# yuzhou42/disinfect-slam

Hardware: AMD Instinct MI355X
Metric: TSDF integrate frames/s (640x480 depth+label, 5mm voxel) (higher is better)
Workload: dtype f32

## Files before the change

### disinfect-slam_amd/csrc/tsdf_device.h

```cpp
#pragma once

#include <hip/hip_runtime.h>
#include <stdint.h>


namespace tsdf {

constexpr int kBlockLenBits = 3;
constexpr int kBlockLen = 8;
constexpr int kBlockVolume = 512;
constexpr int kBlockVolumeBits = 9;
constexpr int kNumBucketBits = 21;
constexpr uint32_t kNumBucket = 1u << kNumBucketBits;
constexpr uint32_t kBucketMask = kNumBucket - 1;
constexpr uint32_t kNumEntry = kNumBucket * 2;
constexpr uint32_t kEntryMask = kNumEntry - 1;
constexpr uint32_t kOccWords = kNumEntry / 64;
constexpr int kBlockBytes = kBlockVolume * 12;
constexpr int kProbOffset = kBlockVolume * 4;
constexpr int kRgbwOffset = kBlockVolume * 8;
constexpr uint32_t kNewKeyCap = 1u << 17;
constexpr int kMaxDdaSamples = 6;
constexpr int64_t kMaxOrderRange = 8192ll * 1024;
constexpr int kResolveThreads = 1024;
// ... 424 lines not shown
  const float u = quot_for_cmp(hx, hz, rz, (float)(P.W - 1));
  const float v = quot_for_cmp(hy, hz, rz, (float)(P.H - 1));
  return u >= 0 && u <= (float)(P.W - 1) && v >= 0 && v <= (float)(P.H - 1) && hz >= 0;
}
template <bool Full>
__device__ __forceinline__ bool block_visible(const FrameParams& P, int16_t bx, int16_t by,
                                              int16_t bz) {
  const int16_t x = (int16_t)(bx << kBlockLenBits), y = (int16_t)(by << kBlockLenBits),
                z = (int16_t)(bz << kBlockLenBits);
  bool vis = Full;
#pragma unroll
  for (int i = 0; i < 8; ++i) {
    const bool v = voxel_visible(P, (int16_t)(x + ((i >> 0) & 1) * (kBlockLen - 1)),
                                 (int16_t)(y + ((i >> 1) & 1) * (kBlockLen - 1)),
                                 (int16_t)(z + ((i >> 2) & 1) * (kBlockLen - 1)));
    if (Full)
      vis = vis && v;
    else
      vis = vis || v;
  }
  return vis;
}

__device__ __forceinline__ f3 pixel_ray(const FrameParams& P, int x, int y) {
  f3 pc;
  pc.x = P.ifx * (float)x + P.icx * 1.0f;
  pc.y = P.ify * (float)y + P.icy * 1.0f;
  pc.z = 1.0f;
  return pc;
}
__device__ __forceinline__ float pixel_w_new(const FrameParams& P, float d) {
  return (1.0f - quot_const(d, P.max_depth, P.inv_max_depth)) * 4.0f;
}

}
```

### disinfect-slam_amd/csrc/tsdf_fuse.hip

```cpp
#include "tsdf_block.h"
#include "tsdf_kernels.h"
#include "tsdf_resolve.h"
#include "tsdf_ingest.h"

namespace tsdf {

__device__ __forceinline__ float comp(const float4& v, int j) {
  return j == 0 ? v.x : j == 1 ? v.y : j == 2 ? v.z : v.w;
}
__device__ __forceinline__ void setc(float4& v, int j, float f) {
  if (j == 0) v.x = f; else if (j == 1) v.y = f; else if (j == 2) v.z = f; else v.w = f;
}
__device__ __forceinline__ uint32_t compu(const uint4& v, int j) {
  return j == 0 ? v.x : j == 1 ? v.y : j == 2 ? v.z : v.w;
}
__device__ __forceinline__ void setu(uint4& v, int j, uint32_t f) {
  if (j == 0) v.x = f; else if (j == 1) v.y = f; else if (j == 2) v.z = f; else v.w = f;
}

__device__ __forceinline__ void frame_end(const EngineDev& D) {
  lds_barrier();
  if (threadIdx.x == 0) {
    D.ctr->total_visible += (unsigned long long)D.ctr->n_vis;
    D.ctr->total_updated += D.ctr->last_updated;
// ... 47 lines not shown

__global__ __launch_bounds__(256) void k_shard_abort(EngineDev D) {
  const int n = min(D.ctr->nk_count, (int)kNewKeyCap);
  for (int i = threadIdx.x; i < n; i += blockDim.x) {
    const int h = (int)D.nk_list[i].slot;
    D.nk_key[h] = 0ull;
    D.nk_order[h] = 0xFFFFFFFFu;
  }
  for (int i = threadIdx.x; i < 3 * kBands; i += blockDim.x) D.band[i * kBandStride] = 0;
  if (threadIdx.x < 2) D.pipe[kPipeNCand + 16 * threadIdx.x] = 0ull;
  for (int i = kPipeStats + threadIdx.x; i < kPipeWords; i += blockDim.x) D.pipe[i] = 0ull;
  for (int i = threadIdx.x; i < kArriveWords; i += blockDim.x) D.arrive[i] = 0ull;
  __syncthreads();
  if (threadIdx.x == 0) {
    D.ctr->nk_count = 0;
    *D.ncand = 0;
    D.ctr->n_fresh = 0;
    D.ctr->n_pend = 0;
    D.ctr->status |= 32u;
  }
}

struct ViewFuse {
  FrameParams R;
  ViewGrid V;
  uint32_t vtag;
};
__device__ __forceinline__ void view_patch_carved(const EngineDev& D, const ViewFuse& F) {
  __builtin_amdgcn_s_waitcnt(0);
  __syncthreads();
  const ViewGrid& V = F.V;
  const int n = min(ld_co(D.ncand), D.cand_cap);
  const int ox = view_origin(F.R.wt.x, F.R.voxel, V.half), oy = view_origin(F.R.wt.y, F.R.voxel, V.half),
            oz = view_origin(F.R.wt.z, F.R.voxel, V.half);
  const unsigned long long* rq = reinterpret_cast<const unsigned long long*>(D.cand);
  for (int k = threadIdx.x; k < n; k += blockDim.x) {
    const unsigned long long a = ld_co(&rq[2 * k]), b = ld_co(&rq[2 * k + 1]);
    const int lx = (int16_t)(a & 0xFFFF) - ox, ly = (int16_t)((a >> 16) & 0xFFFF) - oy,
              lz = (int16_t)((a >> 32) & 0xFFFF) - oz;
    const int32_t idx = (int32_t)(uint32_t)b;
    if ((unsigned)lx >= (unsigned)V.n || (unsigned)ly >= (unsigned)V.n || (unsigned)lz >= (unsigned)V.n || idx < 0)
      continue;
    if (__hip_atomic_load(&D.rtag[idx], __ATOMIC_RELAXED, __HIP_MEMORY_SCOPE_AGENT) != F.vtag) continue;
    const int kb = ((lz >> 2) * V.nb + (ly >> 2)) * V.nb + (lx >> 2);
    __hip_atomic_store(&V.cell[view_cell(kb, lx, ly, lz)], 0u, __ATOMIC_RELAXED, __HIP_MEMORY_SCOPE_AGENT);
  }
}
__device__ __forceinline__ void integrate_tail(const EngineDev& D, const FrameParams& P, DeleteLds& L,
                                               const ViewFuse* F = nullptr) {
  const int t = threadIdx.x;
  const unsigned long long tend = __builtin_amdgcn_s_memrealtime();
  TSDF_STAMP(D, 7, 0);
  if (P.tail == kTailPack)
    pack_cands_wg(D, D.cand, D.ncand, P.slot, P.slot_cap);
  else
    resolve_delete_wg(D, D.cand, D.ncand, 0, L, F ? F->vtag : 0u);
#ifndef TSDF_NO_VIEW_PATCH
  if (F) view_patch_carved(D, *F);
#endif
  TSDF_STAMP(D, 7, 1);
  lds_barrier();
  const int bc = t < kBands ? D.band[t * kBandStride] : 0;
  int nband;
  (void)wg_excl_scan(bc, L.scan, &nband);
  if (t == 0) {
    const unsigned long long upd = arrive_collect(D.arrive + kArrIntegrate);
    D.ctr->last_updated = upd;
    D.ctr->integrate_ticks += tend - ld_co(&D.arrive[kArrStart]);
    D.ctr->n_vis = nband + D.ctr->n_fresh;
  }
  if (P.tail != kTailPack) frame_end(D);
  TSDF_STAMP(D, 7, 2);
}

struct UpdState {
  float4 ts, pr;
  uint4 cw;
  float4 px[4];
  uint32_t pc[4];
  v2f hzs[2];
  bool inb[4];
  bool fresh;
};

__device__ __forceinline__ void update_issue_pool(const EngineDev& D, const VisRec& r, int lane, int hf,
                                                  UpdState& S) {
  const int off = (hf * 256 + lane * 4) * 4;
  const int32_t pidx = r.idx;
  uint8_t* blk = D.pool + (size_t)pidx * kBlockBytes;
  float4& ts = S.ts;
  float4& pr = S.pr;
  uint4& cw = S.cw;
  const bool fresh = r.pad != 0;
  if (fresh) {
    ts = make_float4(-1.f, -1.f, -1.f, -1.f);
    pr = make_float4(0.5f, 0.5f, 0.5f, 0.5f);
    cw = make_uint4(0u, 0u, 0u, 0u);
  } else {
    ts = pool_ld(blk + off);
    pr = pool_ld(blk + kProbOffset + off);
    cw = pool_ldu(blk + kRgbwOffset + off);
  }
  S.fresh = fresh;
}
template <bool Raw>
__device__ __forceinline__ void update_issue_pix(const EngineDev& D, const FrameParams& P, const VisRec& r, int lane,
                                                 int hf, UpdState& S) {
  const int rx0 = (lane & 1) * 4, ry = (lane >> 1) & 7, rz = (lane >> 4) + 4 * hf;
  float4* px = S.px;
  uint32_t* pc = S.pc;
  v2f* hzs = S.hzs;
  bool* inb = S.inb;
  const int16_t ax0 = (int16_t)(r.x << kBlockLenBits), ay = (int16_t)((r.y << kBlockLenBits) + ry),
                az = (int16_t)((r.z << kBlockLenBits) + rz);
  const float fy = (float)ay * P.voxel, fz = (float)az * P.voxel;
  const float qx = P.cq.x, qy = P.cq.y, qz = P.cq.z, qw = P.cq.w;
  const float qx_fz = qx * fz, qx_fy = qx * fy;
  float uvx = qy * fz - qz * fy;
  uvx += uvx;
  const float w_uvx = qw * uvx, qz_uvx = qz * uvx, qy_uvx = qy * uvx;
#pragma unroll
  for (int k = 0; k < 2; ++k) {
    const v2f wx = v2((float)(int16_t)(ax0 + rx0 + 2 * k), (float)(int16_t)(ax0 + rx0 + 2 * k + 1)) * P.voxel;
    v2f uvy = qz * wx - qx_fz;
    v2f uvz = qx_fy - qy * wx;
    uvy += uvy;
    uvz += uvz;
    const v2f cx = qy * uvz - qz * uvy;
    const v2f cy = qz_uvx - qx * uvz;
    const v2f cz = qx * uvy - qy_uvx;
    const v2f pcx = ((wx + w_uvx) + cx) + P.ct.x;
    const v2f pcy = ((fy + qw * uvy) + cy) + P.ct.y;
    const v2f pcz = ((fz + qw * uvz) + cz) + P.ct.z;
    const v2f hx = P.fx * pcx + P.cx * pcz;
    const v2f hy = P.fy * pcy + P.cy * pcz;
    const v2f rz = v2(__builtin_amdgcn_rcpf(pcz.x), __builtin_amdgcn_rcpf(pcz.y));
    int u0, u1, v0, v1;
    round_quot_i2(hx, pcz, rz, true, true, u0, u1);
    round_quot_i2(hy, pcz, rz, true, true, v0, v1);
    hzs[k] = pcz;
    const int uu[2] = {u0, u1}, vv[2] = {v0, v1};
#pragma unroll
    for (int e = 0; e < 2; ++e) {
      const int j = 2 * k + e;
      inb[j] = uu[e] >= 0 && uu[e] < P.W && vv[e] >= 0 && vv[e] < P.H;
      const int img = inb[j] ? vv[e] * P.W + uu[e] : 0;
      if (Raw) {
        pc[j] = (uint32_t)P.rgb[3 * img] | ((uint32_t)P.rgb[3 * img + 1] << 8) |
                ((uint32_t)P.rgb[3 * img + 2] << 16);
        px[j] = make_float4(P.depth[img], P.ht ? P.ht[img] : 1.0f, P.lt ? P.lt[img] : 1.0f,
                            __int_as_float((uu[e] & 0xFFFF) | (vv[e] << 16)));
      } else {
        px[j] = D.pixA[P.pix_off + img];
        pc[j] = D.pixC[P.pix_off + img];
      }
    }
  }
}

template <bool Raw>
__device__ __forceinline__ void update_issue(const EngineDev& D, const FrameParams& P, const VisRec& r, int lane,
                                             int hf, UpdState& S) {
  update_issue_pool(D, r, lane, hf, S);
  update_issue_pix<Raw>(D, P, r, lane, hf, S);
}

template <bool Raw>
__device__ __forceinline__ void update_finish(const EngineDev& D, const FrameParams& P, const VisRec& r, int lane,
                                              int hf, UpdState& S, float& mn, int& my_upd) {
  const int off = (hf * 256 + lane * 4) * 4;
  const float neg_trunc = -P.trunc;
  uint8_t* blk = D.pool + (size_t)r.idx * kBlockBytes;
  float4 ts = S.ts, pr = S.pr;
  uint4 cw = S.cw;
  const float4* px = S.px;
  const uint32_t* pc = S.pc;
  const v2f* hzs = S.hzs;
  const bool* inb = S.inb;
  const bool fresh = S.fresh;
  int upd_mask = 0;
  const uint32_t wold4 = (compu(cw, 0) >> 24) | ((compu(cw, 1) >> 24) << 8) | ((compu(cw, 2) >> 24) << 16) |
                         ((compu(cw, 3) >> 24) << 24);
  float wn[4] = {0.f, 0.f, 0.f, 0.f};
  int pfast = 0;
  v2f lnh2[2], lnl2[2];
#pragma unroll
  for (int k = 0; k < 2; ++k) {
    const int j0 = 2 * k, j1 = 2 * k + 1;
    const v2f d = v2(px[j0].x, px[j1].x);
    v2f rng, w_new = v2(0.f, 0.f), lnh, lnl;
    bool pf0, pf1;
    if (Raw) {
      const int w0 = __float_as_int(px[j0].w), w1 = __float_as_int(px[j1].w);
      const f3 r0 = pixel_ray(P, w0 & 0xFFFF, w0 >> 16);
      const f3 r1 = pixel_ray(P, w1 & 0xFFFF, w1 >> 16);
      rng = v2(sqrtf(dot3(r0, r0)), sqrtf(dot3(r1, r1)));
      w_new = v2(pixel_w_new(P, d.x), pixel_w_new(P, d.y));
      lnh = sem_logf2(v2(px[j0].y, px[j1].y));
      lnl = sem_logf2(v2(px[j0].z, px[j1].z));
      pf0 = sem_pixel_fast(px[j0].y, px[j0].z, d.x, P.max_depth);
      pf1 = sem_pixel_fast(px[j1].y, px[j1].z, d.y, P.max_depth);
    } else {
      rng = v2(fabsf(px[j0].y), fabsf(px[j1].y));
      pf0 = px[j0].y > 0.0f;
      pf1 = px[j1].y > 0.0f;
      lnh = v2(px[j0].z, px[j1].z);
      lnl = v2(px[j0].w, px[j1].w);
    }
    const uint32_t n0 = pc[j0], n1 = pc[j1];
    const v2f sdf = rng * (d - hzs[k]);
    const bool a0 = inb[j0] && !(d.x == 0 || d.x > P.max_depth) && sdf.x > neg_trunc;
    const bool a1 = inb[j1] && !(d.y == 0 || d.y > P.max_depth) && sdf.y > neg_trunc;
    if (a0 || a1) {
      if (!Raw) w_new = (v2(1.0f, 1.0f) - quot_const2(d, P.max_depth, P.inv_max_depth, a0, a1)) * v2(4.0f, 4.0f);
      v2f tn = quot_const2(sdf, P.trunc, P.inv_trunc, a0, a1);
      tn = v2(fminf(1.0f, tn.x), fminf(1.0f, tn.y));
      const uint32_t o0 = compu(cw, j0), o1 = compu(cw, j1);
      const v2f w_old = v2((float)(o0 >> 24), (float)(o1 >> 24));
      const v2f wc = w_old + w_new;
      const v2f iwc = v2(__builtin_amdgcn_rcpf(wc.x), __builtin_amdgcn_rcpf(wc.y));
      uint32_t c0 = 0, c1 = 0;
#pragma unroll
      for (int ch = 0; ch < 3; ++ch) {
        const v2f num = v2((float)((o0 >> (8 * ch)) & 0xFF), (float)((o1 >> (8 * ch)) & 0xFF)) * w_old +
                        v2((float)((n0 >> (8 * ch)) & 0xFF), (float)((n1 >> (8 * ch)) & 0xFF)) * w_new;
        int32_t r0, r1;
        round_quot_pos2(num, wc, iwc, a0, a1, r0, r1);
        c0 |= (uint32_t)min(255, r0) << (8 * ch);
        c1 |= (uint32_t)min(255, r1) << (8 * ch);
      }
      const v2f tnum = v2(comp(ts, j0), comp(ts, j1)) * w_old + tn * w_new;
      const v2f tq = div_pair(tnum, wc, iwc, a0, a1);
      const v2f wr = wc + v2(0x1.fffffep-2f, 0x1.fffffep-2f);
      c0 |= weight_round_cap(wr.x, 40u) << 24;
      c1 |= weight_round_cap(wr.y, 40u) << 24;
      wn[j0] = w_new.x;
      wn[j1] = w_new.y;
      if (a0) {
// ... 39 lines not shown
        const float w_old = (float)((wold4 >> (8 * j)) & 0xFF);
        pn = sem_update_exact(pv, w_old, wn[j], w_old + wn[j], lnh2[j >> 1][j & 1], lnl2[j >> 1][j & 1]);
      }
      setc(pr, j, pn);
    }
  }
  if (upd_mask == 0xF || fresh) {
    pool_st(blk + off, ts);
    pool_st(blk + kProbOffset + off, pr);
    pool_stu(blk + kRgbwOffset + off, cw);
  } else if (upd_mask) {
#pragma unroll
    for (int j = 0; j < 4; ++j)
      if (upd_mask & (1 << j)) {
        reinterpret_cast<float*>(blk + off)[j] = comp(ts, j);
        reinterpret_cast<float*>(blk + kProbOffset + off)[j] = comp(pr, j);
        reinterpret_cast<uint32_t*>(blk + kRgbwOffset + off)[j] = compu(cw, j);
      }
  }
  my_upd += __popc(upd_mask);
}

template <bool Raw>
__device__ __forceinline__ void update_block(const EngineDev& D, const FrameParams& P, const VisRec& r, int lane,
                                             int hf, float& mn, int& my_upd) {
  UpdState S;
  update_issue<Raw>(D, P, r, lane, hf, S);
  update_finish<Raw>(D, P, r, lane, hf, S, mn, my_upd);
}

__device__ __forceinline__ int band_starts_p(const int32_t* band, int lane, int* total) {
  const int c = lane < kBands ? band[lane * kBandStride] : 0;
  int incl = c;
#pragma unroll
  for (int o = 1; o < kBands; o <<= 1) {
    const int n = __shfl_up(incl, o, 64);
    if (lane >= o) incl += n;
  }
  *total = __builtin_amdgcn_readlane(incl, kBands - 1);
  return incl - c;
}
__device__ __forceinline__ int band_starts(const EngineDev& D, int lane, int* total) {
  return band_starts_p(D.band, lane, total);
}
__device__ __forceinline__ size_t band_find_n(int nblocks, int bst, int lane, int b) {
  const unsigned long long m = __ballot(lane < kBands && b >= bst);
  const int bd = __popcll(m) - 1;
  const int ofs = b - __builtin_amdgcn_readlane(bst, bd);
  return (size_t)bd * nblocks + (size_t)__builtin_amdgcn_readfirstlane(ofs);
}
__device__ __forceinline__ size_t band_find(const EngineDev& D, int bst, int lane, int b) {
  return band_find_n(D.nblocks, bst, lane, b);
}

#ifndef TSDF_INTEGRATE_WAVES
#define TSDF_INTEGRATE_WAVES 6
#endif
template <bool Graph, bool Raw>
__device__ __forceinline__ bool integrate_body(const EngineDev& D, const FrameParams& Pv,
                                               const FrameArgs* __restrict__ A, int nint, DeleteLds& L,
                                               int narrive = 0, const ViewFuse* F = nullptr) {
  FrameParams P = Graph ? A->P : Pv;
  if (Graph && A->cands_out) {
    P.tail = kTailPack;
    P.slot = A->cands_out;
    P.slot_cap = A->cand_cap;
  } else if (Graph) {
    P.tail = kTailResolve;
  }
  __shared__ float s_min[4];
  __shared__ int s_upd[4];
  __shared__ int s_last;
  __shared__ int s_ncand, s_ovf;
  __shared__ VisRec s_cand[kIntegrateCandBuf];
  const int lane = lane_id();
  const int wave = __builtin_amdgcn_readfirstlane(threadIdx.x >> 6);
  const int pair = wave >> 1, hf = wave & 1;
  int nvis = 0;
  const int bst = band_starts(D, lane, &nvis);
  const int nband = nvis;
  nvis += D.ctr->n_fresh;
  const int g = blockIdx.x & 7, ngrp = nint >> 3;
  int my_upd = 0;
  if (threadIdx.x == 0) {
    s_ncand = 0;
    s_ovf = 0;
  }
  TSDF_STAMP(D, 3, 0);
  if (blockIdx.x == 0 && threadIdx.x == 0) st_co(&D.arrive[kArrStart], (unsigned long long)__builtin_amdgcn_s_memrealtime());
  const int npairs = (nvis + 1) >> 1;
  const int p_lo = (int)(((long long)npairs * g) >> 3), p_hi = (int)(((long long)npairs * (g + 1)) >> 3);
  for (int pp = p_lo + (blockIdx.x >> 3); pp < p_hi; pp += ngrp) {
    const int b = 2 * pp + pair;
    float mn = __builtin_nanf("");
    VisRec r{};
    if (b < nvis) {
      if (b >= nband) {
        r = D.fresh_vis[b - nband];
      } else {
        r = D.vis[band_find(D, bst, lane, b)];
      }
      update_block<Raw>(D, P, r, lane, hf, mn, my_upd);
    }
    mn = wave_min_u(mn);
    if (lane == 0) s_min[wave] = mn;
    lds_barrier();
    if (hf == 0 && lane == 0 && b < nvis) {
      const float m2 = fminf(s_min[wave], s_min[wave + 1]);
      if (m2 >= 0.9f) {
        const int k = atomicAdd(&s_ncand, 1);
        if (k < kIntegrateCandBuf) {
          s_cand[k] = r;
        } else {
          const int kg = atomicAdd(D.ncand, 1);
          st_rec_co(&D.cand[kg], r);
          s_ovf = 1;
        }
      }
    }
    lds_barrier();
  }
  const int tot = wave_sum(my_upd);
  if (lane == 0) s_upd[wave] = tot;
  lds_barrier();
  const unsigned long long wg_upd = (unsigned long long)(s_upd[0] + s_upd[1] + s_upd[2] + s_upd[3]);
  const int nc = min(s_ncand, kIntegrateCandBuf);
  if (wave == 0 && nc > 0) {
    int k0 = 0;
    if (lane == 0) k0 = atomicAdd(D.ncand, nc);
    k0 = __shfl(k0, 0, 64);
    if (lane < nc) st_rec_co(&D.cand[k0 + lane], s_cand[lane]);
  }
  TSDF_STAMP(D, 3, 1);
#ifdef TSDF_DIAG_STAMPS
  if (threadIdx.x == 0 && D.dbg && blockIdx.x < (unsigned)kDiagMaxWg) {
    unsigned hw, xcc;
    asm volatile("s_getreg_b32 %0, hwreg(HW_REG_HW_ID)" : "=s"(hw));
    asm volatile("s_getreg_b32 %0, hwreg(HW_REG_XCC_ID)" : "=s"(xcc));
    unsigned long long* q = D.dbg + ((size_t)3 * kDiagMaxWg + blockIdx.x) * kDiagStamps;
    q[4] = hw;
    q[5] = xcc;
    q[6] = (unsigned long long)((p_hi - (p_lo + (int)(blockIdx.x >> 3)) + ngrp - 1) / ngrp);
  }
#endif
  const bool drain = (wave == 0 && nc > 0) || (s_ovf && (wave & 1) == 0);
  if (!arrive_last(D.arrive + kArrIntegrate, wg_upd, &s_last, drain, (uint32_t)(narrive ? narrive : nint)))
    return false;
  integrate_tail(D, P, L, F);
  return true;
}

template <bool Graph, bool Raw>
__global__ __launch_bounds__(kIntegrateThreads)
__attribute__((amdgpu_waves_per_eu(TSDF_INTEGRATE_WAVES, TSDF_INTEGRATE_WAVES))) void k_integrate_t(
    EngineDev D, FrameParams Pv, const FrameArgs* __restrict__ A) {
  __shared__ DeleteLds L;
  integrate_body<Graph, Raw>(D, Pv, A, (int)gridDim.x, L);
}

template <bool Graph>
__device__ __forceinline__ void integrate_vg(const EngineDev& D, const FrameParams& Pv, const FrameArgs* A,
                                             const FrameParams& R, const ViewGrid& V, uint32_t vtag, int nint,
                                             DeleteLds& L) {
  const ViewFuse F{R, V, vtag};
  const int narr = (int)gridDim.x;
  if ((int)blockIdx.x < nint) {
    integrate_body<Graph, false>(D, Pv, A, nint, L, narr, &F);
    return;
  }
  const int w = ((int)blockIdx.x - nint) * 256 + (int)threadIdx.x;
  if (V.n && threadIdx.x < 256) {
    const int ox = view_origin(R.wt.x, R.voxel, V.half), oy = view_origin(R.wt.y, R.voxel, V.half),
              oz = view_origin(R.wt.z, R.voxel, V.half);
    unsigned long long occ = D.occ[w];
    while (occ) {
      const int b = __ffsll((long long)occ) - 1;
      occ &= occ - 1;
      const Ent en = load_ent(D.table, (uint32_t)(w * 64 + b));
      const int lx = en.x - ox, ly = en.y - oy, lz = en.z - oz;
      if ((unsigned)lx >= (unsigned)V.n || (unsigned)ly >= (unsigned)V.n || (unsigned)lz >= (unsigned)V.n ||
          !local_idx(en.idx))
        continue;
      const int k = ((lz >> 2) * V.nb + (ly >> 2)) * V.nb + (lx >> 2);
      __hip_atomic_store(&V.cell[view_cell(k, lx, ly, lz)], (V.gen << kViewIdxBits) | (uint32_t)en.idx,
                         __ATOMIC_RELAXED, __HIP_MEMORY_SCOPE_AGENT);
      V.flags[k] = 1;
      V.flags[V.nbw * 32 + ((lz >> 4) * V.ns + (ly >> 4)) * V.ns + (lx >> 4)] = 1;
    }
  }
  __shared__ int s_last;
  if (!arrive_last(D.arrive + kArrIntegrate, 0ull, &s_last, true, (uint32_t)narr)) return;
  if (Graph) {
    FrameParams P = A->P;
    P.tail = kTailResolve;
    integrate_tail(D, P, L, &F);
  } else {
    integrate_tail(D, Pv, L, &F);
  }
}
__global__ __launch_bounds__(kIntegrateThreads)
__attribute__((amdgpu_waves_per_eu(TSDF_INTEGRATE_WAVES, TSDF_INTEGRATE_WAVES))) void k_integrate_vg(
    EngineDev D, FrameParams Pv, FrameParams R, ViewGrid V, uint32_t vtag, int nint) {
  __shared__ DeleteLds L;
  integrate_vg<false>(D, Pv, nullptr, R, V, vtag, nint, L);
}
__global__ __launch_bounds__(kIntegrateThreads)
__attribute__((amdgpu_waves_per_eu(TSDF_INTEGRATE_WAVES, TSDF_INTEGRATE_WAVES))) void k_integrate_vg_g(
    EngineDev D, const FrameArgs* __restrict__ A, int nint) {
  __shared__ DeleteLds L;
  integrate_vg<true>(D, FrameParams{}, A, A->R, A->V, A->vtag, nint, L);
}


__device__ __forceinline__ void pipe_frame_stats(const EngineDev& D, uint32_t f) {
  const int t = threadIdx.x;
  if (t >= 64) return;
  unsigned long long* base = D.pipe + kPipeStats + (size_t)(f & 1u) * (kPipeStatLines * 16);
  const unsigned long long w = base[16 * t], te = base[16 * t + 1];
  base[16 * t] = 0ull;
  base[16 * t + 1] = 0ull;
  unsigned long long vis = w >> 40, upd = w & ((1ull << 40) - 1ull), tmax = te;
#pragma unroll
  for (int o = 32; o > 0; o >>= 1) {
    vis += __shfl_xor(vis, o, 64);
    upd += __shfl_xor(upd, o, 64);
    const unsigned long long m = __shfl_xor(tmax, o, 64);
    tmax = m > tmax ? m : tmax;
  }
  if (t == 0) {
    const unsigned long long t0 = D.pipe[kPipeT0 + 16 * (f & 1u)];
    D.ctr->n_vis = (int32_t)vis;
    D.ctr->last_updated = upd;
    D.ctr->total_visible += vis;
// ... 280 lines not shown
      __builtin_amdgcn_s_sleep(TSDF_PIPE_SLEEP);
      if (++n > (1u << 22)) {
        atomicOr(status, 64u);
        break;
      }
    }
  }
}
__device__ __forceinline__ bool lane_kept(uint32_t* rtag, int32_t idx, uint32_t fc) {
  return __hip_atomic_fetch_or(&rtag[idx], 0u, __ATOMIC_RELAXED, __HIP_MEMORY_SCOPE_AGENT) != fc;
}
__device__ __forceinline__ void pipe_update(const EngineDev& D, const FrameParams& P, const PipeArgs& A, int kind, int wi,
                                            PipeUpdLds& L) {
  int* s_upd = L.upd;
  int* s_vis = L.vis;
  int& s_ncand = L.ncand;
  VisRec* s_cand = L.cand;
  VisRec* s_def = L.def;
  VisRec* s_list = L.list;
  const int lane = lane_id();
  const int wave = __builtin_amdgcn_readfirstlane(threadIdx.x >> 6);
  const int pair = wave >> 1, hf = wave & 1;
  const bool t0 = threadIdx.x == 0;
  const uint32_t fb = A.fid_alloc, fc = A.fid_carve;
  const VisRec* vis = D.vis + (size_t)(fb & 1u) * kBands * (size_t)D.nblocks;
  VisRec* cand = D.cand + (size_t)(fb & 1u) * (size_t)D.cand_cap;
  int32_t* ncand = reinterpret_cast<int32_t*>(D.pipe + kPipeNCand + 16 * (fb & 1u));
  const unsigned long long* carved = D.pipe + kPipeCarved + (blockIdx.x & 7) * 16;
  if (t0) s_ncand = 0;
  if (kind == 0 && wi == 0 && t0)
    st_co(D.pipe + kPipeT0 + 16 * (fb & 1u), (unsigned long long)__builtin_amdgcn_s_memrealtime());
  int bst = 0;
  int nvis = 0, nband = 0, p = 0, p_hi = 0, pstep = 1;
  bool carved_known = false;
  if (kind == 0) {
    bst = band_starts_p(D.band + (size_t)(fb % 3u) * kBands * kBandStride, lane, &nvis);
    nband = nvis;
    if (A.fresh_ready) nvis += D.ctr->n_fresh;
    const int g = wi & 7, npairs = (nvis + 1) >> 1;
    p = (int)(((long long)npairs * g) >> 3) + (wi >> 3);
    p_hi = (int)(((long long)npairs * (g + 1)) >> 3);
    pstep = A.nint >> 3;
  } else {
    wait_tag(D.pipe + kPipeAlloc + (blockIdx.x & 7) * 16, A.tag, &D.ctr->status);
    nvis = ld_co(&D.ctr->n_fresh);
    p = wi;
    p_hi = (nvis + 1) >> 1;
    pstep = kPipeFreshWG;
  }
  const bool chk = A.has_carve && kind == 0;
  const uint32_t* ct = D.ctag + (size_t)(fc & 1u) * D.nblocks;
  int my_upd = 0, my_vis = 0, ndef = 0;
  bool def_done = false;
  const bool fresh_co = kind != 0;
  int& s_n = L.n;
  int& s_ndef = L.ndef;
  float* s_pmin = L.pmin;
  int* s_pdone = L.pdone;
  uint32_t& s_fb = L.fb;
  if (t0) s_fb = fb;
  const unsigned long long lt_mask = (1ull << lane) - 1ull;
  if (t0) s_ndef = 0;
  for (;;) {
    int n = 0;
    lds_barrier();
    if (p < p_hi) {
      const int npr = min((p_hi - p + pstep - 1) / pstep, kPipeList / 2);
      if (wave == 0) {
        const int b = 2 * (p + (lane >> 1) * pstep) + (lane & 1);
        const bool valid = lane < 2 * npr && b < nvis;
        int bd = 0, bs = 0;
#pragma unroll
        for (int k = 1; k < kBands; ++k) {
          const int sk = __builtin_amdgcn_readlane(bst, k);
          if (b >= sk) {
            bd = k;
            bs = sk;
          }
        }
        VisRec r{};
        if (valid) {
          if (b >= nband)
            r = fresh_co ? ld_rec_co(&D.fresh_vis[b - nband]) : D.fresh_vis[b - nband];
          else
            r = vis[(size_t)bd * D.nblocks + (size_t)(b - bs)];
        }
        const bool cand = valid && chk && r.pad == 0 && ct[r.idx] == fc;
        bool take = valid && !cand;
        const unsigned long long cm = __ballot(cand);
        if (cm) {
          const int nc = __popcll(cm);
          if (!carved_known && ndef + nc <= kPipeDefer) {
            if (cand) s_def[ndef + __popcll(cm & lt_mask)] = r;
            ndef += nc;
          } else {
            if (!carved_known) wave_wait_tag(carved, A.tag, &D.ctr->status);
            carved_known = true;
            if (cand) take = lane_kept(D.rtag, r.idx, fc);
          }
        }
        const unsigned long long tm = __ballot(take);
        if (take) s_list[__popcll(tm & lt_mask)] = r;
        s_pdone[lane] = 0;
        if (lane == 0) {
          s_n = __popcll(tm);
          s_ndef = ndef;
        }
      }
      p += npr * pstep;
    } else if (!def_done && s_ndef > 0) {
      if (wave == 0) {
        if (!carved_known) wave_wait_tag(carved, A.tag, &D.ctr->status);
        carved_known = true;
        bool take = false;
        VisRec r{};
        if (lane < ndef) {
          r = s_def[lane];
          take = lane_kept(D.rtag, r.idx, fc);
        }
        const unsigned long long tm = __ballot(take);
        if (take) s_list[__popcll(tm & lt_mask)] = r;
        s_pdone[lane] = 0;
        if (lane == 0) s_n = __popcll(tm);
      }
      def_done = true;
    } else {
      break;
    }
    lds_barrier();
    n = s_n;
#ifdef TSDF_DIAG_STAMPS
    if (t0 && D.dbg && blockIdx.x < (unsigned)kDiagMaxWg) {
      unsigned long long* q = D.dbg + ((size_t)8 * kDiagMaxWg + blockIdx.x) * kDiagStamps;
      const unsigned long long tnow = __builtin_amdgcn_s_memrealtime();
      if (q[5] == 0ull) q[3] = tnow;
      q[4] = tnow;
      q[5] += (unsigned long long)n + 1ull;
    }
#endif
    for (int k = pair; k < n; k += 2) {
      const VisRec r = s_list[k];
      float mn = __builtin_nanf("");
      update_block<false>(D, P, r, lane, hf, mn, my_upd);
      my_vis += hf == 0 ? 1 : 0;
      mn = wave_min_u(mn);
      if (lane == 0) {
        s_pmin[2 * k + hf] = mn;
        __builtin_amdgcn_fence(__ATOMIC_RELEASE, "workgroup", "local");
        if (atomicAdd(&s_pdone[k], 1) == 1) {
          __builtin_amdgcn_fence(__ATOMIC_ACQUIRE, "workgroup", "local");
          const float m2 = fminf(mn, s_pmin[2 * k + (hf ^ 1)]);
          if (m2 >= 0.9f) {
            const uint32_t f = s_fb;
            D.ctag[(size_t)(f & 1u) * D.nblocks + r.idx] = f;
            const int kc = atomicAdd(&s_ncand, 1);
            if (kc < kIntegrateCandBuf) {
              s_cand[kc] = r;
            } else {
              const int kg = atomicAdd(ncand, 1);
              if (kg < D.cand_cap) st_rec_co(&cand[kg], r);
              else atomicOr(&D.ctr->status, 16u);
            }
          }
        }
      }
    }
  }
  const int tot = wave_sum(my_upd);
  if (lane == 0) {
    s_upd[wave] = tot;
    s_vis[wave] = my_vis;
  }
  lds_barrier();
  const int nc = min(s_ncand, kIntegrateCandBuf);
  if (wave == 0 && nc > 0) {
    int k0 = 0;
    if (lane == 0) k0 = atomicAdd(ncand, nc);
    k0 = __shfl(k0, 0, 64);
    if (lane < nc && k0 + lane < D.cand_cap) st_rec_co(&cand[k0 + lane], s_cand[lane]);
  }
  if (t0) {
    const unsigned long long upd = (unsigned long long)(s_upd[0] + s_upd[1] + s_upd[2] + s_upd[3]);
    const unsigned long long nv = (unsigned long long)(s_vis[0] + s_vis[1] + s_vis[2] + s_vis[3]);
    unsigned long long* st = D.pipe + kPipeStats + (size_t)(fb & 1u) * (kPipeStatLines * 16) +
// ... 66 lines not shown
  } else
    vis_sweep_chained<1024>(frame_view(D, A.fid_new), Pn, o, U.ing, aflag, A.tag);
  if (threadIdx.x == 0)
    atomicMax(D.pipe + kPipeIngEnd + 16 * (A.fid_new & 1u), (unsigned long long)__builtin_amdgcn_s_memrealtime());
  return 3 + part;
}
__device__ __forceinline__ void frame_body(const EngineDev& D, const FrameParams& Pu, const FrameParams& Pn,
                                           const PipeArgs& A, FrameLds& U) {
#ifdef TSDF_DIAG_STAMPS
  const unsigned long long d_t0 = __builtin_amdgcn_s_memrealtime();
#endif
  const int code = frame_part(D, Pu, Pn, A, U);
#ifdef TSDF_DIAG_STAMPS
  if (threadIdx.x == 0 && D.dbg && blockIdx.x < (unsigned)kDiagMaxWg) {
    unsigned long long* q = D.dbg + ((size_t)8 * kDiagMaxWg + blockIdx.x) * kDiagStamps;
    q[0] = (unsigned long long)code;
    q[1] = d_t0;
    q[2] = __builtin_amdgcn_s_memrealtime();
  }
#else
  (void)code;
#endif
}
__global__ __launch_bounds__(kIntegrateThreads)
__attribute__((amdgpu_waves_per_eu(TSDF_FRAME_WAVES, TSDF_FRAME_WAVES))) void k_frame(
    EngineDev D, FrameParams Pu, FrameParams Pn, PipeArgs A) {
  __shared__ FrameLds U;
  frame_body(D, Pu, Pn, A, U);
}
__global__ __launch_bounds__(kIntegrateThreads)
__attribute__((amdgpu_waves_per_eu(TSDF_FRAME_WAVES, TSDF_FRAME_WAVES))) void k_frame_g(
    EngineDev D, const FrameArgs* __restrict__ FA) {
  __shared__ FrameLds U;
  const PipeArgs A = FA->pipe;
  const FrameParams Pu = FA->Pu, Pn = FA->P;
  frame_body(D, Pu, Pn, A, U);
}

template __global__ void k_integrate_t<false, false>(EngineDev, FrameParams, const FrameArgs*);
template __global__ void k_integrate_t<true, false>(EngineDev, FrameParams, const FrameArgs*);
template __global__ void k_integrate_t<false, true>(EngineDev, FrameParams, const FrameArgs*);
template __global__ void k_integrate_t<true, true>(EngineDev, FrameParams, const FrameArgs*);

__device__ __forceinline__ void merge_cands_inbox(const EngineDev& D, VisRec* cand, int32_t* ncand, const ShardRec* __restrict__ cands_in,
                                  int cap, int nshard, int* s_base) {
  if (threadIdx.x == 0) {
    int run = 0;
    bool ovf = false;
    for (int s = 0; s < nshard; ++s) {
      s_base[s] = run;
      int n = min((int)cands_in[(size_t)s * (cap + 1)].val, cap);
      if (n > D.cand_cap - run) {
        n = D.cand_cap - run;
        ovf = true;
      }
      run += n;
    }
    s_base[nshard] = run;
    st_co(ncand, run);
// ... 47 lines not shown
```

Measured before the change: 24820.

## Pin frame constants in scalar registers and read kernel args in place

Gathers the per-frame constants and base pointers used by the voxel update into a struct, and uses empty inline asm to force them into scalar registers. Kernel parameters are now read by reference from the kernarg segment instead of being copied into registers or stack, and the per-lane in-bounds bool array becomes a bitmask. ViewFuse holds references instead of copies. The aim is to lower VGPR and scratch pressure and drop redundant loads in the hot integrate loops. The risk is that forcing values into scalar registers raises SGPR pressure or constrains scheduling.

```diff
diff --git a/disinfect-slam_amd/csrc/tsdf_device.h b/disinfect-slam_amd/csrc/tsdf_device.h
--- a/disinfect-slam_amd/csrc/tsdf_device.h
+++ b/disinfect-slam_amd/csrc/tsdf_device.h
@@ -470,15 +470,21 @@
   return vis;
 }
 
-__device__ __forceinline__ f3 pixel_ray(const FrameParams& P, int x, int y) {
+__device__ __forceinline__ f3 pixel_ray(float ifx, float ify, float icx, float icy, int x, int y) {
   f3 pc;
-  pc.x = P.ifx * (float)x + P.icx * 1.0f;
-  pc.y = P.ify * (float)y + P.icy * 1.0f;
+  pc.x = ifx * (float)x + icx * 1.0f;
+  pc.y = ify * (float)y + icy * 1.0f;
   pc.z = 1.0f;
   return pc;
 }
+__device__ __forceinline__ f3 pixel_ray(const FrameParams& P, int x, int y) {
+  return pixel_ray(P.ifx, P.ify, P.icx, P.icy, x, y);
+}
+__device__ __forceinline__ float pixel_w_new(float max_depth, float inv_max_depth, float d) {
+  return (1.0f - quot_const(d, max_depth, inv_max_depth)) * 4.0f;
+}
 __device__ __forceinline__ float pixel_w_new(const FrameParams& P, float d) {
-  return (1.0f - quot_const(d, P.max_depth, P.inv_max_depth)) * 4.0f;
-}
-
-}
+  return pixel_w_new(P.max_depth, P.inv_max_depth, d);
+}
+
+}
diff --git a/disinfect-slam_amd/csrc/tsdf_fuse.hip b/disinfect-slam_amd/csrc/tsdf_fuse.hip
--- a/disinfect-slam_amd/csrc/tsdf_fuse.hip
+++ b/disinfect-slam_amd/csrc/tsdf_fuse.hip
@@ -93,8 +93,8 @@
 }
 
 struct ViewFuse {
-  FrameParams R;
-  ViewGrid V;
+  const FrameParams& R;
+  const ViewGrid& V;
   uint32_t vtag;
 };
 __device__ __forceinline__ void view_patch_carved(const EngineDev& D, const ViewFuse& F) {
@@ -117,13 +117,13 @@
     __hip_atomic_store(&V.cell[view_cell(kb, lx, ly, lz)], 0u, __ATOMIC_RELAXED, __HIP_MEMORY_SCOPE_AGENT);
   }
 }
-__device__ __forceinline__ void integrate_tail(const EngineDev& D, const FrameParams& P, DeleteLds& L,
+__device__ __forceinline__ void integrate_tail(const EngineDev& D, int tail, ShardRec* slot, int slot_cap, DeleteLds& L,
                                                const ViewFuse* F = nullptr) {
   const int t = threadIdx.x;
   const unsigned long long tend = __builtin_amdgcn_s_memrealtime();
   TSDF_STAMP(D, 7, 0);
-  if (P.tail == kTailPack)
-    pack_cands_wg(D, D.cand, D.ncand, P.slot, P.slot_cap);
+  if (tail == kTailPack)
+    pack_cands_wg(D, D.cand, D.ncand, slot, slot_cap);
   else
     resolve_delete_wg(D, D.cand, D.ncand, 0, L, F ? F->vtag : 0u);
 #ifndef TSDF_NO_VIEW_PATCH
@@ -140,7 +140,7 @@
     D.ctr->integrate_ticks += tend - ld_co(&D.arrive[kArrStart]);
     D.ctr->n_vis = nband + D.ctr->n_fresh;
   }
-  if (P.tail != kTailPack) frame_end(D);
+  if (tail != kTailPack) frame_end(D);
   TSDF_STAMP(D, 7, 2);
 }
 
@@ -150,15 +150,76 @@
   float4 px[4];
   uint32_t pc[4];
   v2f hzs[2];
-  bool inb[4];
+  int inb;
   bool fresh;
 };
 
-__device__ __forceinline__ void update_issue_pool(const EngineDev& D, const VisRec& r, int lane, int hf,
+struct UpdConst {
+  uint8_t* pool;
+  const float4* pixA;
+  const uint32_t* pixC;
+  const float* depth;
+  const uint8_t* rgb;
+  const float* ht;
+  const float* lt;
+  float ifx, ify, icx, icy;
+  int W, H;
+  float voxel;
+  quatf cq;
+  f3 ct;
+  float fx, fy, cx, cy;
+  float trunc, neg_trunc, inv_trunc, max_depth, inv_max_depth;
+};
+template <typename T>
+__device__ __forceinline__ T uniform_reg(T v) {
+  asm("" : "+s"(v));
+  return v;
+}
+template <typename T>
+__device__ __forceinline__ T* uniform_reg(T* p) {
+  auto g = (__attribute__((address_space(1))) T*)p;
+  asm("" : "+s"(g));
+  return (T*)g;
+}
+template <bool Raw>
+__device__ __forceinline__ UpdConst upd_const(const EngineDev& D, const FrameParams& P) {
+  UpdConst C{};
+  C.pool = uniform_reg(D.pool);
+  if (Raw) {
+    C.depth = uniform_reg(P.depth);
+    C.rgb = uniform_reg(P.rgb);
+    C.ht = uniform_reg(P.ht);
+    C.lt = uniform_reg(P.lt);
+    C.ifx = uniform_reg(P.ifx);
+    C.ify = uniform_reg(P.ify);
+    C.icx = uniform_reg(P.icx);
+    C.icy = uniform_reg(P.icy);
+  } else {
+    C.pixA = uniform_reg(D.pixA + P.pix_off);
+    C.pixC = uniform_reg(D.pixC + P.pix_off);
+  }
+  C.W = uniform_reg(P.W);
+  C.H = uniform_reg(P.H);
+  C.voxel = uniform_reg(P.voxel);
+  C.cq = {uniform_reg(P.cq.x), uniform_reg(P.cq.y), uniform_reg(P.cq.z), uniform_reg(P.cq.w)};
+  C.ct = {uniform_reg(P.ct.x), uniform_reg(P.ct.y), uniform_reg(P.ct.z)};
+  C.fx = uniform_reg(P.fx);
+  C.fy = uniform_reg(P.fy);
+  C.cx = uniform_reg(P.cx);
+  C.cy = uniform_reg(P.cy);
+  C.trunc = uniform_reg(P.trunc);
+  C.neg_trunc = -C.trunc;
+  C.inv_trunc = uniform_reg(P.inv_trunc);
+  C.max_depth = uniform_reg(P.max_depth);
+  C.inv_max_depth = uniform_reg(P.inv_max_depth);
+  return C;
+}
+
+__device__ __forceinline__ void update_issue_pool(const UpdConst& C, const VisRec& r, int lane, int hf,
                                                   UpdState& S) {
   const int off = (hf * 256 + lane * 4) * 4;
   const int32_t pidx = r.idx;
-  uint8_t* blk = D.pool + (size_t)pidx * kBlockBytes;
+  uint8_t* blk = C.pool + (size_t)pidx * kBlockBytes;
   float4& ts = S.ts;
   float4& pr = S.pr;
   uint4& cw = S.cw;
@@ -175,24 +236,23 @@
   S.fresh = fresh;
 }
 template <bool Raw>
-__device__ __forceinline__ void update_issue_pix(const EngineDev& D, const FrameParams& P, const VisRec& r, int lane,
-                                                 int hf, UpdState& S) {
+__device__ __forceinline__ void update_issue_pix(const UpdConst& C, const VisRec& r, int lane, int hf, UpdState& S) {
   const int rx0 = (lane & 1) * 4, ry = (lane >> 1) & 7, rz = (lane >> 4) + 4 * hf;
   float4* px = S.px;
   uint32_t* pc = S.pc;
   v2f* hzs = S.hzs;
-  bool* inb = S.inb;
+  int inb = 0;
   const int16_t ax0 = (int16_t)(r.x << kBlockLenBits), ay = (int16_t)((r.y << kBlockLenBits) + ry),
                 az = (int16_t)((r.z << kBlockLenBits) + rz);
-  const float fy = (float)ay * P.voxel, fz = (float)az * P.voxel;
-  const float qx = P.cq.x, qy = P.cq.y, qz = P.cq.z, qw = P.cq.w;
+  const float fy = (float)ay * C.voxel, fz = (float)az * C.voxel;
+  const float qx = C.cq.x, qy = C.cq.y, qz = C.cq.z, qw = C.cq.w;
   const float qx_fz = qx * fz, qx_fy = qx * fy;
   float uvx = qy * fz - qz * fy;
   uvx += uvx;
   const float w_uvx = qw * uvx, qz_uvx = qz * uvx, qy_uvx = qy * uvx;
 #pragma unroll
   for (int k = 0; k < 2; ++k) {
-    const v2f wx = v2((float)(int16_t)(ax0 + rx0 + 2 * k), (float)(int16_t)(ax0 + rx0 + 2 * k + 1)) * P.voxel;
+    const v2f wx = v2((float)(int16_t)(ax0 + rx0 + 2 * k), (float)(int16_t)(ax0 + rx0 + 2 * k + 1)) * C.voxel;
     v2f uvy = qz * wx - qx_fz;
     v2f uvz = qx_fy - qy * wx;
     uvy += uvy;
@@ -200,11 +260,11 @@
     const v2f cx = qy * uvz - qz * uvy;
     const v2f cy = qz_uvx - qx * uvz;
     const v2f cz = qx * uvy - qy_uvx;
-    const v2f pcx = ((wx + w_uvx) + cx) + P.ct.x;
-    const v2f pcy = ((fy + qw * uvy) + cy) + P.ct.y;
-    const v2f pcz = ((fz + qw * uvz) + cz) + P.ct.z;
-    const v2f hx = P.fx * pcx + P.cx * pcz;
-    const v2f hy = P.fy * pcy + P.cy * pcz;
+    const v2f pcx = ((wx + w_uvx) + cx) + C.ct.x;
+    const v2f pcy = ((fy + qw * uvy) + cy) + C.ct.y;
+    const v2f pcz = ((fz + qw * uvz) + cz) + C.ct.z;
+    const v2f hx = C.fx * pcx + C.cx * pcz;
+    const v2f hy = C.fy * pcy + C.cy * pcz;
     const v2f rz = v2(__builtin_amdgcn_rcpf(pcz.x), __builtin_amdgcn_rcpf(pcz.y));
     int u0, u1, v0, v1;
     round_quot_i2(hx, pcz, rz, true, true, u0, u1);
@@ -214,40 +274,41 @@
 #pragma unroll
     for (int e = 0; e < 2; ++e) {
       const int j = 2 * k + e;
-      inb[j] = uu[e] >= 0 && uu[e] < P.W && vv[e] >= 0 && vv[e] < P.H;
-      const int img = inb[j] ? vv[e] * P.W + uu[e] : 0;
+      const bool in = uu[e] >= 0 && uu[e] < C.W && vv[e] >= 0 && vv[e] < C.H;
+      inb |= in ? 1 << j : 0;
+      const int img = in ? vv[e] * C.W + uu[e] : 0;
       if (Raw) {
-        pc[j] = (uint32_t)P.rgb[3 * img] | ((uint32_t)P.rgb[3 * img + 1] << 8) |
-                ((uint32_t)P.rgb[3 * img + 2] << 16);
-        px[j] = make_float4(P.depth[img], P.ht ? P.ht[img] : 1.0f, P.lt ? P.lt[img] : 1.0f,
+        pc[j] = (uint32_t)C.rgb[3 * img] | ((uint32_t)C.rgb[3 * img + 1] << 8) |
+                ((uint32_t)C.rgb[3 * img + 2] << 16);
+        px[j] = make_float4(C.depth[img], C.ht ? C.ht[img] : 1.0f, C.lt ? C.lt[img] : 1.0f,
                             __int_as_float((uu[e] & 0xFFFF) | (vv[e] << 16)));
       } else {
-        px[j] = D.pixA[P.pix_off + img];
-        pc[j] = D.pixC[P.pix_off + img];
+        px[j] = C.pixA[img];
+        pc[j] = C.pixC[img];
       }
     }
   }
+  S.inb = inb;
 }
 
 template <bool Raw>
-__device__ __forceinline__ void update_issue(const EngineDev& D, const FrameParams& P, const VisRec& r, int lane,
-                                             int hf, UpdState& S) {
-  update_issue_pool(D, r, lane, hf, S);
-  update_issue_pix<Raw>(D, P, r, lane, hf, S);
+__device__ __forceinline__ void update_issue(const UpdConst& C, const VisRec& r, int lane, int hf, UpdState& S) {
+  update_issue_pool(C, r, lane, hf, S);
+  update_issue_pix<Raw>(C, r, lane, hf, S);
 }
 
 template <bool Raw>
-__device__ __forceinline__ void update_finish(const EngineDev& D, const FrameParams& P, const VisRec& r, int lane,
-                                              int hf, UpdState& S, float& mn, int& my_upd) {
+__device__ __forceinline__ void update_finish(const UpdConst& C, const VisRec& r, int lane, int hf, UpdState& S,
+                                              float& mn, int& my_upd) {
   const int off = (hf * 256 + lane * 4) * 4;
-  const float neg_trunc = -P.trunc;
-  uint8_t* blk = D.pool + (size_t)r.idx * kBlockBytes;
+  const float neg_trunc = C.neg_trunc;
+  uint8_t* blk = C.pool + (size_t)r.idx * kBlockBytes;
   float4 ts = S.ts, pr = S.pr;
   uint4 cw = S.cw;
   const float4* px = S.px;
   const uint32_t* pc = S.pc;
   const v2f* hzs = S.hzs;
-  const bool* inb = S.inb;
+  const int inb = S.inb;
   const bool fresh = S.fresh;
   int upd_mask = 0;
   const uint32_t wold4 = (compu(cw, 0) >> 24) | ((compu(cw, 1) >> 24) << 8) | ((compu(cw, 2) >> 24) << 16) |
@@ -263,14 +324,14 @@
     bool pf0, pf1;
     if (Raw) {
       const int w0 = __float_as_int(px[j0].w), w1 = __float_as_int(px[j1].w);
-      const f3 r0 = pixel_ray(P, w0 & 0xFFFF, w0 >> 16);
-      const f3 r1 = pixel_ray(P, w1 & 0xFFFF, w1 >> 16);
+      const f3 r0 = pixel_ray(C.ifx, C.ify, C.icx, C.icy, w0 & 0xFFFF, w0 >> 16);
+      const f3 r1 = pixel_ray(C.ifx, C.ify, C.icx, C.icy, w1 & 0xFFFF, w1 >> 16);
       rng = v2(sqrtf(dot3(r0, r0)), sqrtf(dot3(r1, r1)));
-      w_new = v2(pixel_w_new(P, d.x), pixel_w_new(P, d.y));
+      w_new = v2(pixel_w_new(C.max_depth, C.inv_max_depth, d.x), pixel_w_new(C.max_depth, C.inv_max_depth, d.y));
       lnh = sem_logf2(v2(px[j0].y, px[j1].y));
       lnl = sem_logf2(v2(px[j0].z, px[j1].z));
-      pf0 = sem_pixel_fast(px[j0].y, px[j0].z, d.x, P.max_depth);
-      pf1 = sem_pixel_fast(px[j1].y, px[j1].z, d.y, P.max_depth);
+      pf0 = sem_pixel_fast(px[j0].y, px[j0].z, d.x, C.max_depth);
+      pf1 = sem_pixel_fast(px[j1].y, px[j1].z, d.y, C.max_depth);
     } else {
       rng = v2(fabsf(px[j0].y), fabsf(px[j1].y));
       pf0 = px[j0].y > 0.0f;
@@ -280,11 +341,11 @@
     }
     const uint32_t n0 = pc[j0], n1 = pc[j1];
     const v2f sdf = rng * (d - hzs[k]);
-    const bool a0 = inb[j0] && !(d.x == 0 || d.x > P.max_depth) && sdf.x > neg_trunc;
-    const bool a1 = inb[j1] && !(d.y == 0 || d.y > P.max_depth) && sdf.y > neg_trunc;
+    const bool a0 = ((inb >> j0) & 1) && !(d.x == 0 || d.x > C.max_depth) && sdf.x > neg_trunc;
+    const bool a1 = ((inb >> j1) & 1) && !(d.y == 0 || d.y > C.max_depth) && sdf.y > neg_trunc;
     if (a0 || a1) {
-      if (!Raw) w_new = (v2(1.0f, 1.0f) - quot_const2(d, P.max_depth, P.inv_max_depth, a0, a1)) * v2(4.0f, 4.0f);
-      v2f tn = quot_const2(sdf, P.trunc, P.inv_trunc, a0, a1);
+      if (!Raw) w_new = (v2(1.0f, 1.0f) - quot_const2(d, C.max_depth, C.inv_max_depth, a0, a1)) * v2(4.0f, 4.0f);
+      v2f tn = quot_const2(sdf, C.trunc, C.inv_trunc, a0, a1);
       tn = v2(fminf(1.0f, tn.x), fminf(1.0f, tn.y));
       const uint32_t o0 = compu(cw, j0), o1 = compu(cw, j1);
       const v2f w_old = v2((float)(o0 >> 24), (float)(o1 >> 24));
@@ -370,11 +431,11 @@
 }
 
 template <bool Raw>
-__device__ __forceinline__ void update_block(const EngineDev& D, const FrameParams& P, const VisRec& r, int lane,
-                                             int hf, float& mn, int& my_upd) {
+__device__ __forceinline__ void update_block(const UpdConst& C, const VisRec& r, int lane, int hf, float& mn,
+                                             int& my_upd) {
   UpdState S;
-  update_issue<Raw>(D, P, r, lane, hf, S);
-  update_finish<Raw>(D, P, r, lane, hf, S, mn, my_upd);
+  update_issue<Raw>(C, r, lane, hf, S);
+  update_finish<Raw>(C, r, lane, hf, S, mn, my_upd);
 }
 
 __device__ __forceinline__ int band_starts_p(const int32_t* band, int lane, int* total) {
@@ -408,14 +469,7 @@
 __device__ __forceinline__ bool integrate_body(const EngineDev& D, const FrameParams& Pv,
                                                const FrameArgs* __restrict__ A, int nint, DeleteLds& L,
                                                int narrive = 0, const ViewFuse* F = nullptr) {
-  FrameParams P = Graph ? A->P : Pv;
-  if (Graph && A->cands_out) {
-    P.tail = kTailPack;
-    P.slot = A->cands_out;
-    P.slot_cap = A->cand_cap;
-  } else if (Graph) {
-    P.tail = kTailResolve;
-  }
+  const FrameParams& P = Graph ? A->P : Pv;
   __shared__ float s_min[4];
   __shared__ int s_upd[4];
   __shared__ int s_last;
@@ -438,17 +492,23 @@
   if (blockIdx.x == 0 && threadIdx.x == 0) st_co(&D.arrive[kArrStart], (unsigned long long)__builtin_amdgcn_s_memrealtime());
   const int npairs = (nvis + 1) >> 1;
   const int p_lo = (int)(((long long)npairs * g) >> 3), p_hi = (int)(((long long)npairs * (g + 1)) >> 3);
+  const UpdConst C = upd_const<Raw>(D, P);
+  const VisRec* vis = uniform_reg(D.vis);
+  const VisRec* fresh_vis = uniform_reg(D.fresh_vis);
+  const int nblocks = uniform_reg(D.nblocks);
+  VisRec* cand = uniform_reg(D.cand);
+  int32_t* ncand = uniform_reg(D.ncand);
   for (int pp = p_lo + (blockIdx.x >> 3); pp < p_hi; pp += ngrp) {
     const int b = 2 * pp + pair;
     float mn = __builtin_nanf("");
     VisRec r{};
     if (b < nvis) {
       if (b >= nband) {
-        r = D.fresh_vis[b - nband];
+        r = fresh_vis[b - nband];
       } else {
-        r = D.vis[band_find(D, bst, lane, b)];
+        r = vis[band_find_n(nblocks, bst, lane, b)];
       }
-      update_block<Raw>(D, P, r, lane, hf, mn, my_upd);
+      update_block<Raw>(C, r, lane, hf, mn, my_upd);
     }
     mn = wave_min_u(mn);
     if (lane == 0) s_min[wave] = mn;
@@ -460,8 +520,8 @@
         if (k < kIntegrateCandBuf) {
           s_cand[k] = r;
         } else {
-          const int kg = atomicAdd(D.ncand, 1);
-          st_rec_co(&D.cand[kg], r);
+          const int kg = atomicAdd(ncand, 1);
+          st_rec_co(&cand[kg], r);
           s_ovf = 1;
         }
       }
@@ -494,16 +554,31 @@
   const bool drain = (wave == 0 && nc > 0) || (s_ovf && (wave & 1) == 0);
   if (!arrive_last(D.arrive + kArrIntegrate, wg_upd, &s_last, drain, (uint32_t)(narrive ? narrive : nint)))
     return false;
-  integrate_tail(D, P, L, F);
+  if (Graph && A->cands_out)
+    integrate_tail(D, kTailPack, A->cands_out, A->cand_cap, L, F);
+  else if (Graph)
+    integrate_tail(D, kTailResolve, nullptr, 0, L, F);
+  else
+    integrate_tail(D, P.tail, P.slot, P.slot_cap, L, F);
   return true;
 }
 
+template <typename T>
+__device__ __forceinline__ const T& kernel_args() {
+  return *(const T*)(const __attribute__((address_space(4))) T*)__builtin_amdgcn_kernarg_segment_ptr();
+}
+struct IntegrateKernArgs {
+  EngineDev D;
+  FrameParams Pv;
+  const FrameArgs* A;
+};
 template <bool Graph, bool Raw>
 __global__ __launch_bounds__(kIntegrateThreads)
 __attribute__((amdgpu_waves_per_eu(TSDF_INTEGRATE_WAVES, TSDF_INTEGRATE_WAVES))) void k_integrate_t(
     EngineDev D, FrameParams Pv, const FrameArgs* __restrict__ A) {
   __shared__ DeleteLds L;
-  integrate_body<Graph, Raw>(D, Pv, A, (int)gridDim.x, L);
+  const IntegrateKernArgs& K = kernel_args<IntegrateKernArgs>();
+  integrate_body<Graph, Raw>(K.D, K.Pv, A, (int)gridDim.x, L);
 }
 
 template <bool Graph>
@@ -538,25 +613,31 @@
   }
   __shared__ int s_last;
   if (!arrive_last(D.arrive + kArrIntegrate, 0ull, &s_last, true, (uint32_t)narr)) return;
-  if (Graph) {
-    FrameParams P = A->P;
-    P.tail = kTailResolve;
-    integrate_tail(D, P, L, &F);
-  } else {
-    integrate_tail(D, Pv, L, &F);
-  }
-}
+  if (Graph)
+    integrate_tail(D, kTailResolve, nullptr, 0, L, &F);
+  else
+    integrate_tail(D, Pv.tail, Pv.slot, Pv.slot_cap, L, &F);
+}
+struct IntegrateVgKernArgs {
+  EngineDev D;
+  FrameParams Pv, R;
+  ViewGrid V;
+  uint32_t vtag;
+  int nint;
+};
 __global__ __launch_bounds__(kIntegrateThreads)
 __attribute__((amdgpu_waves_per_eu(TSDF_INTEGRATE_WAVES, TSDF_INTEGRATE_WAVES))) void k_integrate_vg(
     EngineDev D, FrameParams Pv, FrameParams R, ViewGrid V, uint32_t vtag, int nint) {
   __shared__ DeleteLds L;
-  integrate_vg<false>(D, Pv, nullptr, R, V, vtag, nint, L);
+  const IntegrateVgKernArgs& K = kernel_args<IntegrateVgKernArgs>();
+  integrate_vg<false>(K.D, K.Pv, nullptr, K.R, K.V, vtag, nint, L);
 }
 __global__ __launch_bounds__(kIntegrateThreads)
 __attribute__((amdgpu_waves_per_eu(TSDF_INTEGRATE_WAVES, TSDF_INTEGRATE_WAVES))) void k_integrate_vg_g(
     EngineDev D, const FrameArgs* __restrict__ A, int nint) {
   __shared__ DeleteLds L;
-  integrate_vg<true>(D, FrameParams{}, A, A->R, A->V, A->vtag, nint, L);
+  const EngineDev& Dk = kernel_args<EngineDev>();
+  integrate_vg<true>(Dk, A->P, A, A->R, A->V, A->vtag, nint, L);
 }
 
 
@@ -883,7 +964,7 @@
   const int wave = __builtin_amdgcn_readfirstlane(threadIdx.x >> 6);
   const int pair = wave >> 1, hf = wave & 1;
   const bool t0 = threadIdx.x == 0;
-  const uint32_t fb = A.fid_alloc, fc = A.fid_carve;
+  const uint32_t fb = uniform_reg(A.fid_alloc), fc = uniform_reg(A.fid_carve);
   const VisRec* vis = D.vis + (size_t)(fb & 1u) * kBands * (size_t)D.nblocks;
   VisRec* cand = D.cand + (size_t)(fb & 1u) * (size_t)D.cand_cap;
   int32_t* ncand = reinterpret_cast<int32_t*>(D.pipe + kPipeNCand + 16 * (fb & 1u));
@@ -922,6 +1003,13 @@
   if (t0) s_fb = fb;
   const unsigned long long lt_mask = (1ull << lane) - 1ull;
   if (t0) s_ndef = 0;
+  const UpdConst C = upd_const<false>(D, P);
+  const VisRec* fresh_vis = uniform_reg(D.fresh_vis);
+  const int nblocks = uniform_reg(D.nblocks), cand_cap = uniform_reg(D.cand_cap);
+  uint32_t* rtag = uniform_reg(D.rtag);
+  uint32_t* ctag_b = uniform_reg(D.ctag + (size_t)(fb & 1u) * D.nblocks);
+  uint32_t* status = uniform_reg(&D.ctr->status);
+  const uint32_t tag = uniform_reg(A.tag);
   for (;;) {
     int n = 0;
     lds_barrier();
@@ -942,9 +1030,9 @@
         VisRec r{};
         if (valid) {
           if (b >= nband)
-            r = fresh_co ? ld_rec_co(&D.fresh_vis[b - nband]) : D.fresh_vis[b - nband];
+            r = fresh_co ? ld_rec_co(&fresh_vis[b - nband]) : fresh_vis[b - nband];
           else
-            r = vis[(size_t)bd * D.nblocks + (size_t)(b - bs)];
+            r = vis[(size_t)bd * nblocks + (size_t)(b - bs)];
         }
         const bool cand = valid && chk && r.pad == 0 && ct[r.idx] == fc;
         bool take = valid && !cand;
@@ -955,9 +1043,9 @@
             if (cand) s_def[ndef + __popcll(cm & lt_mask)] = r;
             ndef += nc;
           } else {
-            if (!carved_known) wave_wait_tag(carved, A.tag, &D.ctr->status);
+            if (!carved_known) wave_wait_tag(carved, tag, status);
             carved_known = true;
-            if (cand) take = lane_kept(D.rtag, r.idx, fc);
+            if (cand) take = lane_kept(rtag, r.idx, fc);
           }
         }
         const unsigned long long tm = __ballot(take);
@@ -971,13 +1059,13 @@
       p += npr * pstep;
     } else if (!def_done && s_ndef > 0) {
       if (wave == 0) {
-        if (!carved_known) wave_wait_tag(carved, A.tag, &D.ctr->status);
+        if (!carved_known) wave_wait_tag(carved, tag, status);
         carved_known = true;
         bool take = false;
         VisRec r{};
         if (lane < ndef) {
           r = s_def[lane];
-          take = lane_kept(D.rtag, r.idx, fc);
+          take = lane_kept(rtag, r.idx, fc);
         }
         const unsigned long long tm = __ballot(take);
         if (take) s_list[__popcll(tm & lt_mask)] = r;
@@ -999,11 +1087,11 @@
       q[5] += (unsigned long long)n + 1ull;
     }
 #endif
+    if (hf == 0 && n > pair) my_vis += (n - pair + 1) >> 1;
     for (int k = pair; k < n; k += 2) {
       const VisRec r = s_list[k];
       float mn = __builtin_nanf("");
-      update_block<false>(D, P, r, lane, hf, mn, my_upd);
-      my_vis += hf == 0 ? 1 : 0;
+      update_block<false>(C, r, lane, hf, mn, my_upd);
       mn = wave_min_u(mn);
       if (lane == 0) {
         s_pmin[2 * k + hf] = mn;
@@ -1013,14 +1101,14 @@
           const float m2 = fminf(mn, s_pmin[2 * k + (hf ^ 1)]);
           if (m2 >= 0.9f) {
             const uint32_t f = s_fb;
-            D.ctag[(size_t)(f & 1u) * D.nblocks + r.idx] = f;
+            ctag_b[r.idx] = f;
             const int kc = atomicAdd(&s_ncand, 1);
             if (kc < kIntegrateCandBuf) {
               s_cand[kc] = r;
             } else {
               const int kg = atomicAdd(ncand, 1);
-              if (kg < D.cand_cap) st_rec_co(&cand[kg], r);
-              else atomicOr(&D.ctr->status, 16u);
+              if (kg < cand_cap) st_rec_co(&cand[kg], r);
+              else atomicOr(status, 16u);
             }
           }
         }
@@ -1133,19 +1221,23 @@
   (void)code;
 #endif
 }
+struct FrameKernArgs {
+  EngineDev D;
+  FrameParams Pu, Pn;
+  PipeArgs A;
+};
 __global__ __launch_bounds__(kIntegrateThreads)
 __attribute__((amdgpu_waves_per_eu(TSDF_FRAME_WAVES, TSDF_FRAME_WAVES))) void k_frame(
     EngineDev D, FrameParams Pu, FrameParams Pn, PipeArgs A) {
   __shared__ FrameLds U;
-  frame_body(D, Pu, Pn, A, U);
+  const FrameKernArgs& K = kernel_args<FrameKernArgs>();
+  frame_body(K.D, K.Pu, K.Pn, K.A, U);
 }
 __global__ __launch_bounds__(kIntegrateThreads)
 __attribute__((amdgpu_waves_per_eu(TSDF_FRAME_WAVES, TSDF_FRAME_WAVES))) void k_frame_g(
     EngineDev D, const FrameArgs* __restrict__ FA) {
   __shared__ FrameLds U;
-  const PipeArgs A = FA->pipe;
-  const FrameParams Pu = FA->Pu, Pn = FA->P;
-  frame_body(D, Pu, Pn, A, U);
+  frame_body(kernel_args<EngineDev>(), FA->Pu, FA->P, FA->pipe, U);
 }
 
 template __global__ void k_integrate_t<false, false>(EngineDev, FrameParams, const FrameArgs*);
```

Result: faster. 25740, median of 6 (+3.7%).
